# cdcseacave/openMVS

Measured on AMD Instinct MI355X. Metric: Mpix/s depth-map output at 1920x1080 N-view, higher is better.
Workload: dtype f32

## Files before the change

### openmvs_amd/csrc/pm_band.hip

```cpp
#pragma once

#ifndef PM_NDRAW
#define PM_NDRAW 6
#endif
#ifndef PM_BAND_MINWAVES
#define PM_BAND_MINWAVES 3
#endif
#ifndef PM_BAND_MINWAVES_PHOTO
#define PM_BAND_MINWAVES_PHOTO 4
#endif

struct alignas(16) PMPix {
	float nb[2][5];
	float depth, nx, ny, nz, conf;
	float p0, p1, scaleRange, depthRange;
	int st, it, idxScale, flags;
	float hd, hnx, hny, hnz, hp0, hp1;
	int hst, pad0;
	float qX[4][3], qn[4][3];
	float vx, vy, normSq0, sumW;
	double X0x, X0y;
	int x, y;
	float x1[2];
	double hr[3];
	float dr[PM_NDRAW][3];
};
#if defined(__HIP_DEVICE_COMPILE__)
#define PM_LDS __attribute__((address_space(3)))
template <class T> __device__ __forceinline__ PM_LDS T* pm_launder(T* p) { PM_LDS T* q = (PM_LDS T*)p; asm volatile("" : "+v"(q)); return q; }
#else
#define PM_LDS
template <class T> __device__ __forceinline__ T* pm_launder(T* p) { return p; }
#endif
static_assert(sizeof(PMPix) == 368, "sixteen of them, the weights and the views' matrices fit a sixteenth of a CU's LDS (tests/test_kernel_resources.py)");
__device__ __forceinline__ PM_LDS float* pm_pix_sf(PM_LDS PMPix* P) { return P->nb[0]; }
enum { PMF_SMOOTH = 1, PMF_CHANGED = 2, PMF_POK0 = 4, PMF_POK1 = 8 };

template <int G, int VPL, bool GEO, bool BUF, bool TILED>
__device__ __forceinline__ void pm_visit(const PMTask& t, const PMKParams& kp, const PMImgBuf& rs, uint32_t pass, int sgn, float2* s_wg, PMPix* s_pixg, const double* hotBase,
		int g, int v, bool active, int x, int y, int ySafe, size_t idx, const bool* bok, const int* qxs, const int* qys, const size_t* qis, unsigned oldMask,
		float n0D, float n0N0, float n0N1, float n0N2, float n0C, float n1D, float n1N0, float n1N1, float n1N2, float n1C,
		float& rD, float& rN0, float& rN1, float& rN2, float& rC, bool& wr PM_PROF_ARG) {
	constexpr int NBD = PM_SRC_HOT + (GEO ? PM_SRC_GEO : 0);
	constexpr int PPW = 64 / G;
	const int slot = v & 3;
	const pm_gf gDepth = pm_globw(t.depth), gNormal = pm_globw(t.normal), gConf = pm_globw(t.conf);
	const int yTop = ySafe;
	float oDepth = 0.f, oNx = 0.f, oNy = 0.f, oNz = 0.f, oConf = 2.f, prior = 0.f;
	float myD = 0.f, myN0 = 0.f, myN1 = 0.f, myN2 = 1.f;
	unsigned char maskByte = 1;
	if (active && v < 4) {
		if (v == 0) {
			if (t.prior) prior = pm_glob(t.prior)[idx];
			if (t.mask != nullptr) maskByte = t.mask[idx];
			oDepth = gDepth[idx]; oNx = gNormal[idx * 3]; oNy = gNormal[idx * 3 + 1]; oNz = gNormal[idx * 3 + 2]; oConf = gConf[idx];
			myD = bok[0] ? n0D : 0.f; myN0 = n0N0; myN1 = n0N1; myN2 = n0N2;
		}
		else if (v == 1) { myD = bok[1] ? n1D : 0.f; myN0 = n1N0; myN1 = n1N1; myN2 = n1N2; }
		else {
			const size_t qi = slot == 2 ? qis[2] : qis[3];
			const bool old = TILED && ((oldMask >> slot) & 1u);
			const pm_gcf sD = pm_glob(old ? t.depthOld : t.depth), sN = pm_glob(old ? t.normalOld : t.normal);
// ... 103 lines not shown
					else {
						const PmPhilox4 r = pm_philox4x32_10((uint32_t)px, (uint32_t)py, (uint32_t)(PM_STREAM_REFINE * 256) + it, 0u, t.k0, k1);
						e0 = 2.f * pm_u32_to_unit(r.v[0]) - 1.f; e1 = 2.f * pm_u32_to_unit(r.v[1]) - 1.f; e2 = 2.f * pm_u32_to_unit(r.v[2]) - 1.f;
					}
					++it;
					const float ndepth = P->depth + (depthRange * scaleRange) * e0;
					if (!pm_in_range(ndepth, t.dMin, t.dMax)) continue;
					hp0 = p0 + (kp.angle1Range * scaleRange) * e1;
					hp1 = p1 + (kp.angle2Range * scaleRange) * e2;
					pm_dir2normal_vm<PPW>(hp0, hp1, v, hnx, hny, hnz);
					if (hnx * vx + hny * vy + hnz * vz >= 0) continue;
					hd = ndepth;
					need = true; hst = ST_REFINE;
				}
			}
			double hr0 = 0.0, hr1 = 0.0, hr2 = 0.0;
			if (need) pm_homography_plane(P->X0x, P->X0y, hd, hnx, hny, hnz, hr0, hr1, hr2);
			__builtin_amdgcn_wave_barrier();
			if (v == 0) {
				P->hr[0] = hr0; P->hr[1] = hr1; P->hr[2] = hr2;
				P->st = st; P->it = (int)it; P->idxScale = (int)idxScale; P->flags = flags;
				P->scaleRange = scaleRange; P->depthRange = depthRange; P->p0 = p0; P->p1 = p1;
				P->hd = hd; P->hnx = hnx; P->hny = hny; P->hnz = hnz; P->hp0 = hp0; P->hp1 = hp1; P->hst = hst;
			}
		}
		const unsigned long long needBal = __ballot(need);
		if (needBal == 0ull) break;
		PM_TICK(1); PM_COUNT(8, __popcll(needBal)); PM_HIST(__popcll(needBal) / G);
		typename std::conditional<GEO, PMGeoReq, PMNoGeoReq>::type greq[GEO ? VPL : 1];
		if constexpr (GEO) {
			const PM_LDS PMPix* P = pm_launder(s_pixg);
			const double gX0x = P->X0x, gX0y = P->X0y;
#pragma unroll
			for (int u = 0; u < VPL; ++u) {
				const int vw = v + u * G;
				PM_CENSUS_GEO(vw);
				pm_geo_request(need && vw < t.nSrc, hotBase + vw * NBD + PM_SRC_HOT, gX0x, gX0y, hd, greq[u]);
			}
			PM_CENSUS_GEO(-1);
			PM_GEO_HOLD();
		}
		{
			PM_LDS PMPix* P = pm_launder(s_pixg);
			const int flags = P->flags;
			const bool on = need && v < 4 && (flags & PMF_SMOOTH) && ((flags >> (8 + slot)) & 1);
			float myF = 1.f;
// ... 3 lines not shown
				const float planeD = -hd * (hnx * vx + hny * vy + hnz * 1.f);
				const float dist = (hnx * q0 + (hny * q1 + hnz * q2)) + planeD;
				const float r = dist / hd;
				const float factorDepth = pm_expf((r * r) * kp.smoothSigmaDepth);
				const float ca = pm_clampf((hnx * m0 + hny * m1 + hnz * m2) / pm_sqrtf((hnx * hnx + hny * hny + hnz * hnz) * (m0 * m0 + m1 * m1 + m2 * m2)), -1.f, 1.f);
				const float ac = pm_acosf(ca);
				const float factorNormal = pm_expf((ac * ac) * kp.smoothSigmaNormal);
				myF = (1.f - kp.smoothBonusDepth * factorDepth) * (1.f - kp.smoothBonusNormal * factorNormal);
			}
			if (v < 4) pm_pix_sf(P)[slot] = myF;
			__builtin_amdgcn_wave_barrier();
		}
		PM_TICK(2);
		float sc = PM_INF, sc2 = PM_INF;
		{
			const PM_LDS PMPix* P = pm_launder(s_pixg);
#pragma unroll 1
			for (int u = 0; u < VPL; ++u) {
				const int vw = v + u * G;
				if (need && vw < t.nSrc) {
					PM_CENSUS_VIEW(t.w, G, u);
					float s1;
					if constexpr (GEO) s1 = pm_score_view<GEO, BUF ? 2 : 1, true, true>(t.src[vw], t, kp, P->x, P->y, P->X0x, P->X0y, P->normSq0, P->sumW, s_wg, hd, hnx, hny, hnz, 1.f, 1.f, 1.f, 1.f, 0.f,
						hotBase + vw * NBD, hotBase + vw * NBD + PM_SRC_HOT, rs PM_PROF_PASS, (const double*)P->hr, (const float*)pm_pix_sf((PM_LDS PMPix*)P), greq, u, VPL);
					else s1 = pm_score_view<GEO, BUF ? 2 : 1, true, true>(t.src[vw], t, kp, P->x, P->y, P->X0x, P->X0y, P->normSq0, P->sumW, s_wg, hd, hnx, hny, hnz, 1.f, 1.f, 1.f, 1.f, 0.f,
						hotBase + vw * NBD, hotBase + vw * NBD + PM_SRC_HOT, rs PM_PROF_PASS, (const double*)P->hr, (const float*)pm_pix_sf((PM_LDS PMPix*)P));
					PM_CENSUS_VIEW_END();
					if (s1 < sc) { sc2 = sc; sc = s1; } else if (s1 < sc2) sc2 = s1;
				}
			}
		}
		const float nconf = pm_aggregate_vm<G>(sc, t.nSrc, kp.thRobust, sc2);
		{
			PM_LDS PMPix* P = pm_launder(s_pixg);
			if (need && v == 0 && P->conf > nconf) {
				P->conf = nconf; P->depth = P->hd; P->nx = P->hnx; P->ny = P->hny; P->nz = P->hnz;
				int flags = P->flags | PMF_CHANGED;
				P->flags = flags;
				const int hst = P->hst;
				if (hst == ST_RAND) { if (nconf < kp.thConfRand) P->st = ST_DECIDE; }
				else if (hst == ST_REFINE) { P->p0 = P->hp0; P->p1 = P->hp1; const int is = P->idxScale + 1; P->idxScale = is; P->scaleRange = pm_pow2neg((unsigned)is); }
			}
		}
		__builtin_amdgcn_wave_barrier();
		PM_TICK(6);
	}
	{
		const PM_LDS PMPix* P = pm_launder(s_pixg);
		wr = (P->flags & PMF_CHANGED) && valid;
		rD = wr ? P->depth : oDepth; rN0 = wr ? P->nx : oNx; rN1 = wr ? P->ny : oNy; rN2 = wr ? P->nz : oNz; rC = wr ? P->conf : oConf;
	}
}

template <int G, int VPL, bool GEO, bool BUF, bool TILED>
__global__ __launch_bounds__(64, (GEO ? PM_BAND_MINWAVES : PM_BAND_MINWAVES_PHOTO)) void pm_sweep2_kernel(const PMTask* __restrict__ tasks, PMKParams kp, PMStep st, uint32_t pass) {
	constexpr int PPW = 64 / G;
	constexpr int NV = G * VPL;
	constexpr int NBD = PM_SRC_HOT + (GEO ? PM_SRC_GEO : 0);
	static_assert(G >= 4, "a pixel gets at least a quad of lanes");
	PM_PROF_DECL;
	__shared__ float2 s_w[PPW][PM_NT + 1];
	__shared__ double s_src[NV * NBD];
	__shared__ PMPix s_pix[PPW];
	unsigned vbx = blockIdx.x, vby = blockIdx.y;
	{
		const unsigned nbx = gridDim.x, nwg = nbx * gridDim.y, orig = blockIdx.y * nbx + blockIdx.x;
		const unsigned xcd = orig % 8u, q = nwg / 8u, r = nwg % 8u;
		const unsigned wgid = (xcd < r ? xcd * (q + 1u) : r * (q + 1u) + (xcd - r) * q) + orig / 8u;
		vby = wgid / nbx; vbx = wgid - vby * nbx;
	}
	const PMTask& t = tasks[vby];
	const PMImgBuf rs = pm_make_imgbuf(t);
	const int lane = threadIdx.x;
	for (int i = lane; i < NV * NBD; i += 64) {
		double e = ((const double*)&t.src[i / NBD])[i % NBD];
		if constexpr (GEO) if (i % NBD == PM_SRC_HOT + 12) {
			const PMSrcView& sv = t.src[i / NBD];
			const float4* q = sv.depth != nullptr ? pm_task_geoq(t) + sv.dqBase : nullptr;
			e = *(const double*)&q;
		}
		s_src[i] = e;
	}
	const int g = lane % PPW, v = lane / PPW;
	const int w = t.w, h = t.h;
	const PMStepPix sp = pm_step_pixel<TILED>(st, w, h, (int)vbx * PPW + g);
	const bool active = sp.active;
	const int x = sp.x, y = sp.y;
	const size_t idx = (size_t)y * w + x;
	const int sgn = st.dir == 0 ? -1 : 1;
	bool bok[4]; int qxs[4], qys[4]; size_t qis[4];
#pragma unroll
	for (int k = 0; k < 4; ++k) {
		const int ox = (k == 0) ? sgn : (k == 2 ? -sgn : 0), oy = (k == 1) ? sgn : (k == 3 ? -sgn : 0);
		bool ok;
		if (ox == -1) ok = x > PM_HW; else if (ox == 1) ok = x < w - PM_HW; else if (oy == -1) ok = y > PM_HW; else ok = y < h - PM_HW;
		bok[k] = ok && active; qxs[k] = x + ox; qys[k] = y + oy;
		qis[k] = bok[k] ? (size_t)(y + oy) * w + (x + ox) : idx;
	}
	const pm_gf gDepth = pm_globw(t.depth), gNormal = pm_globw(t.normal), gConf = pm_globw(t.conf);
	float n0D = 0.f, n0N0 = 0.f, n0N1 = 0.f, n0N2 = 0.f, n0C = 2.f, n1D = 0.f, n1N0 = 0.f, n1N1 = 0.f, n1N2 = 0.f, n1C = 2.f;
	if (active && v < 2) {
		const size_t q0 = qis[0], q1 = qis[1];
		if (TILED) {
			const pm_gcf nD0 = pm_glob((sp.oldMask & 1u) ? t.depthOld : t.depth), nN0 = pm_glob((sp.oldMask & 1u) ? t.normalOld : t.normal), nC0 = pm_glob((sp.oldMask & 1u) ? t.confOld : t.conf);
			const pm_gcf nD1 = pm_glob((sp.oldMask & 2u) ? t.depthOld : t.depth), nN1 = pm_glob((sp.oldMask & 2u) ? t.normalOld : t.normal), nC1 = pm_glob((sp.oldMask & 2u) ? t.confOld : t.conf);
			if (v == 0) { n0D = nD0[q0]; n0N0 = nN0[q0 * 3]; n0N1 = nN0[q0 * 3 + 1]; n0N2 = nN0[q0 * 3 + 2]; n0C = nC0[q0]; }
			else { n1D = nD1[q1]; n1N0 = nN1[q1 * 3]; n1N1 = nN1[q1 * 3 + 1]; n1N2 = nN1[q1 * 3 + 2]; n1C = nC1[q1]; }
		} else {
			if (v == 0) { n0D = gDepth[q0]; n0N0 = gNormal[q0 * 3]; n0N1 = gNormal[q0 * 3 + 1]; n0N2 = gNormal[q0 * 3 + 2]; n0C = gConf[q0]; }
			else { n1D = gDepth[q1]; n1N0 = gNormal[q1 * 3]; n1N1 = gNormal[q1 * 3 + 1]; n1N2 = gNormal[q1 * 3 + 2]; n1C = gConf[q1]; }
		}
	}
	__syncthreads();
	float rD, rN0, rN1, rN2, rC; bool wr;
	pm_visit<G, VPL, GEO, BUF, TILED>(t, kp, rs, pass, sgn, s_w[g], &s_pix[g], s_src, g, v, active, x, y, active ? y : PM_HW, active ? idx : (size_t)PM_HW * w + PM_HW, bok, qxs, qys, qis, sp.oldMask,
		n0D, n0N0, n0N1, n0N2, n0C, n1D, n1N0, n1N1, n1N2, n1C, rD, rN0, rN1, rN2, rC, wr PM_PROF_PASS);
	if (wr && v == 0) { gDepth[idx] = rD; gNormal[idx * 3] = rN0; gNormal[idx * 3 + 1] = rN1; gNormal[idx * 3 + 2] = rN2; gConf[idx] = rC; }
	PM_PROF_FLUSH();
}
```

### openmvs_amd/csrc/pm_kernels.hip

```cpp
#pragma once
#include <hip/hip_runtime.h>
#include <cstddef>
#include <type_traits>
#include "pm_math.h"

#define PM_MAX_SRC 16
#ifndef PM_BLOCK
#define PM_BLOCK 64
#endif
typedef const float __attribute__((address_space(1)))* pm_gcf;
typedef float __attribute__((address_space(1)))* pm_gf;
#if defined(__HIP_DEVICE_COMPILE__)
typedef float pm_f4v __attribute__((ext_vector_type(4)));
typedef const pm_f4v __attribute__((address_space(1)))* pm_gcf4;
__device__ __forceinline__ pm_gcf4 pm_glob4(const float4* p) { return (pm_gcf4)p; }
__device__ __forceinline__ pm_f4v pm_loadq(pm_gcf4 base, unsigned off) { return base[off]; }
#else
typedef const float4* pm_gcf4;
__device__ __forceinline__ pm_gcf4 pm_glob4(const float4* p) { return p; }
__device__ __forceinline__ float4 pm_loadq(pm_gcf4 base, unsigned off) { return base[off]; }
#endif
__device__ __forceinline__ pm_gcf pm_glob(const float* p) { return (pm_gcf)p; }
__device__ __forceinline__ pm_gf pm_globw(float* p) { return (pm_gf)p; }
#define PM_HW 4
// ... 84 lines not shown
#define PM_COUNT(i, n) do { _pa.a[i] += (unsigned long long)(n); } while (0)
#define PM_HIST(n) do { const int _n = (n); if ((threadIdx.x & 63) == 0) atomicAdd(&pm_hist[_n > 16 ? 16 : _n], 1ull); } while (0)
#define PM_PROF_FLUSH() do { if ((threadIdx.x & 63) == 0) for (int _i = 0; _i < 16; ++_i) atomicAdd(&pm_prof[_i], _pa.a[_i]); } while (0)
#else
#define PM_PROF_ARG
#define PM_PROF_PASS
#define PM_PROF_DECL do {} while (0)
#define PM_TICK(i) do {} while (0)
#define PM_COUNT(i, n) do {} while (0)
#define PM_HIST(n) do {} while (0)
#define PM_PROF_FLUSH() do {} while (0)
#endif
#define PM_FD2R(d) ((d) * (PM_PI_F / 180.f))

#if defined(__HIP_DEVICE_COMPILE__)
__device__ __forceinline__ int pm_mul24(int a, int b) { return __mul24(a, b); }
#else
__device__ __forceinline__ int pm_mul24(int a, int b) { return (int)((unsigned)a * (unsigned)b); }
#endif
__device__ __forceinline__ bool pm_inside1(float px, float py, int w, int h) {
	return px >= 1.f && py >= 1.f && px <= (float)(w - 2) && py <= (float)(h - 2);
}
__device__ __forceinline__ bool pm_in_range(float d, float lo, float hi) { return lo <= d && d < hi; }

__device__ __forceinline__ void pm_dir2normal(float p0, float p1, float& nx, float& ny, float& nz) {
	float sx, cx, sy, cy;
	pm_sincosf(p0, &sx, &cx); pm_sincosf(p1, &sy, &cy);
	nx = cx * sy; ny = sx * sy; nz = cy;
}
__device__ __forceinline__ void pm_random_normal(float u1, float u2, float vx, float vy, float vz, float& nx, float& ny, float& nz) {
	const float a0 = PM_FD2R(0.f), a1 = PM_FD2R(180.f), b0 = PM_FD2R(90.f), b1 = PM_FD2R(180.f);
	const float p0 = a0 + (a1 - a0) * u1;
	const float p1 = b0 + (b1 - b0) * u2;
	pm_dir2normal(p0, p1, nx, ny, nz);
	if (nx * vx + ny * vy + nz * vz > 0) { nx = -nx; ny = -ny; nz = -nz; }
}
__device__ __forceinline__ void pm_correct_normal(float vx, float vy, float vz, float& nx, float& ny, float& nz) {
	const float cosAngLen = nx * vx + ny * vy + nz * vz;
	if (cosAngLen >= 0) {
		const float nv = pm_sqrtf(vx * vx + vy * vy + vz * vz);
		const float phi = pm_minf((pm_acosf(pm_clampf(cosAngLen / nv, -1.f, 1.f)) - PM_FD2R(90.f)) * 1.01f, -0.001f);
		float a0 = ny * vz - nz * vy, a1 = nz * vx - nx * vz, a2 = nx * vy - ny * vx;
		const float an = pm_sqrtf(a0 * a0 + a1 * a1 + a2 * a2);
		const float ia = 1.f / an;
		a0 *= ia; a1 *= ia; a2 *= ia;
		float s, c; pm_sincosf(phi, &s, &c);
// ... 245 lines not shown
	q0 = i0 < r.count ? r.base[i0] : z; q1 = i1 < r.count ? r.base[i1] : z; q2 = i2 < r.count ? r.base[i2] : z; q3 = i3 < r.count ? r.base[i3] : z; q4 = i4 < r.count ? r.base[i4] : z;
}
template <int LEFT> __device__ __forceinline__ void pm_bufwait5(pm_f4v&, pm_f4v&, pm_f4v&, pm_f4v&, pm_f4v&) {}
__device__ __forceinline__ unsigned pm_mad24(int a, int b, unsigned c) { return (unsigned)(((unsigned)a & 0xffffffu) * ((unsigned)b & 0xffffffu)) + c; }
#endif

#ifndef PM_CENSUS_TRIP
#define PM_CENSUS_TRIP()
#define PM_CENSUS_GEO(vw)
#define PM_CENSUS_VIEW(width, G, u)
#define PM_CENSUS_VIEW_AS(width, G, u, lane)
#define PM_CENSUS_VIEW_END()
#endif
#ifdef PM_PROBE_WIDEN_QUAD_BLOCK
struct PMImgBuf { pm_rsrc rs; bool oneBlock = false; };
#else
struct PMImgBuf { pm_rsrc rs; };
#endif
__device__ __forceinline__ PMImgBuf pm_make_imgbuf(const PMTask& t) {
	PMImgBuf b;
	b.rs = pm_make_rsrc(t.qArr, t.qCount);
	return b;
}

template <bool QUAD>
__device__ __forceinline__ void pm_tap_row_global(const pm_gcf img, int sw, int sh, float h0, float h3, float h6, float X0, float X1, float X2,
		const float2* wrow, float& sum, float& sumSq, float& num, bool& oob)
{
	const int lxMax = sw - 2, lyMax = sh - 2;
	float fxs[5], fys[5];
	unsigned offs[5];
#pragma unroll
	for (int j = 0; j < 5; ++j) {
		float ptx, pty;
		pm_div2(X0, X1, X2, &ptx, &pty);
		oob = oob || !pm_inside1(ptx, pty, sw, sh);
		int lx = (int)ptx, ly = (int)pty;
		fxs[j] = ptx - (float)lx; fys[j] = pty - (float)ly;
		lx = min(max(lx, 0), lxMax); ly = min(max(ly, 0), lyMax);
		offs[j] = QUAD ? 4u * ((unsigned)(lx + ly) * (unsigned)sh + (unsigned)ly) : (unsigned)ly * (unsigned)sw + (unsigned)lx;
		X0 += h0; X1 += h3; X2 += h6;
	}
	float v00[5], v01[5], v10[5], v11[5];
#pragma unroll
	for (int j = 0; j < 5; ++j) {
		const pm_gcf p = img + offs[j];
		if (QUAD) { v00[j] = p[0]; v01[j] = p[1]; v10[j] = p[2]; v11[j] = p[3]; }
		else { v00[j] = p[0]; v01[j] = p[1]; v10[j] = p[sw]; v11[j] = p[sw + 1]; }
	}
#pragma unroll
	for (int j = 0; j < 5; ++j) {
		const float fx = fxs[j], fx1 = 1.f - fx, fy = fys[j], fy1 = 1.f - fy;
		const float v = (v00[j] * fx1 + v01[j] * fx) * fy1 + (v10[j] * fx1 + v11[j] * fx) * fy;
		const float2 pw = wrow[j];
		const float vw = v * pw.x;
		sum += vw;
		sumSq += v * vw;
		num += v * pw.y;
	}
}

struct PMRowPos { float ptx[5], pty[5]; };
struct PMRowQ { pm_f4v q0, q1, q2, q3, q4; };
struct PMTapRange { int zlo, zhi, plo, pxhi, pyhi; };
__device__ __forceinline__ void pm_range_corner(PMTapRange& rg, float px, float py, float z) {
	const int ix = pm_f2i(px), iy = pm_f2i(py), iz = pm_f2i(z);
	rg.plo = min(rg.plo, min(ix, iy)); rg.pxhi = max(rg.pxhi, ix); rg.pyhi = max(rg.pyhi, iy);
	rg.zlo = min(rg.zlo, iz); rg.zhi = max(rg.zhi, iz);
}
template <bool BUF, bool CORNERS>
__device__ __forceinline__ void pm_row_issue(const PMImgBuf& rs, unsigned qbase, const pm_gcf4 imgQ, int sw, int sh, float h0, float h3, float h6, float X0, float X1, float X2,
		PMRowPos& p, PMRowQ& q, PMTapRange& rg)
{
	unsigned idx[5];
#pragma unroll
	for (int j = 0; j < 5; ++j) {
		pm_div2_inrange(X0, X1, X2, &p.ptx[j], &p.pty[j]);
		const int lx = (int)p.ptx[j], ly = (int)p.pty[j];
		if (BUF) idx[j] = pm_mad24(lx, sh, pm_mad24(ly, sh + 1, qbase));
		else { const int lxc = min(max(lx, 0), sw - 2), lyc = min(max(ly, 0), sh - 2); idx[j] = (unsigned)(lxc + lyc) * (unsigned)sh + (unsigned)lyc; }
		if (CORNERS && (j == 0 || j == 4)) pm_range_corner(rg, p.ptx[j], p.pty[j], X2);
		X0 += h0; X1 += h3; X2 += h6;
	}
#if defined(PM_PROBE_WIDEN_QUAD_BLOCK) && defined(__HIP_DEVICE_COMPILE__)
	if (BUF && rs.oneBlock) {
#pragma unroll
		for (int j = 0; j < 5; ++j) idx[j] = (idx[j] & 3u) | ((unsigned)__builtin_amdgcn_update_dpp((int)idx[j], (int)idx[j], 0x00, 0xf, 0xf, false) & ~3u);
	}
#endif
	if (BUF) pm_bufload5(q.q0, q.q1, q.q2, q.q3, q.q4, idx[0], idx[1], idx[2], idx[3], idx[4], rs.rs);
	else { q.q0 = pm_loadq(imgQ, idx[0]); q.q1 = pm_loadq(imgQ, idx[1]); q.q2 = pm_loadq(imgQ, idx[2]); q.q3 = pm_loadq(imgQ, idx[3]); q.q4 = pm_loadq(imgQ, idx[4]); }
}
template <bool BUF, int LEFT>
__device__ __forceinline__ void pm_row_consume(const PMRowPos& p, PMRowQ& q, const float2* wrow, float& sum, float& sumSq, float& num)
{
	float t00[5], t01[5], t10[5], t11[5];
	if (BUF) pm_bufwait5<LEFT>(q.q0, q.q1, q.q2, q.q3, q.q4);
	const pm_f4v qq[5] = {q.q0, q.q1, q.q2, q.q3, q.q4};
#pragma unroll
	for (int j = 0; j < 5; ++j) { t00[j] = qq[j].x; t01[j] = qq[j].y; t10[j] = qq[j].z; t11[j] = qq[j].w; }
#pragma unroll
	for (int j = 0; j < 5; ++j) {
		const float fx = pm_fract_pos(p.ptx[j]), fx1 = 1.f - fx, fy = pm_fract_pos(p.pty[j]), fy1 = 1.f - fy;
		const float v = (t00[j] * fx1 + t01[j] * fx) * fy1 + (t10[j] * fx1 + t11[j] * fx) * fy;
		const float2 pw = wrow[j];
		const float vw = v * pw.x;
		sum += vw;
		sumSq += v * vw;
		num += v * pw.y;
	}
}
template <bool BUF>
__device__ __forceinline__ void pm_taps_fast(const PMImgBuf& rs, unsigned qbase, const pm_gcf4 imgQ, int sw, int sh, const float* H, float bX0, float bX1, float bX2,
		const float2* wts, float& sum, float& sumSq, float& num, PMTapRange& rg)
{
	PMRowPos pa, pb; PMRowQ qa, qb;
	pm_row_issue<BUF, true>(rs, qbase, imgQ, sw, sh, H[0], H[3], H[6], bX0, bX1, bX2, pa, qa, rg);
#pragma unroll 1
	for (int i = 0; i < 4; i += 2) {
		bX0 += H[1]; bX1 += H[4]; bX2 += H[7];
		pm_row_issue<BUF, false>(rs, qbase, imgQ, sw, sh, H[0], H[3], H[6], bX0, bX1, bX2, pb, qb, rg);
		PM_SCHED_BARRIER();
		pm_row_consume<BUF, 5>(pa, qa, wts + i * 5, sum, sumSq, num);
		PM_SCHED_BARRIER();
		bX0 += H[1]; bX1 += H[4]; bX2 += H[7];
		pm_row_issue<BUF, false>(rs, qbase, imgQ, sw, sh, H[0], H[3], H[6], bX0, bX1, bX2, pa, qa, rg);
		PM_SCHED_BARRIER();
		pm_row_consume<BUF, 5>(pb, qb, wts + (i + 1) * 5, sum, sumSq, num);
		PM_SCHED_BARRIER();
	}
	pm_range_corner(rg, pa.ptx[0], pa.pty[0], bX2);
	pm_range_corner(rg, pa.ptx[4], pa.pty[4], (((bX2 + H[6]) + H[6]) + H[6]) + H[6]);
	pm_row_consume<BUF, 0>(pa, qa, wts + 20, sum, sumSq, num);
}

#if !defined(__HIP_DEVICE_COMPILE__) && defined(PM_DEBUG_REDO)
inline unsigned long long pm_tap_census[2][4];
extern "C" __attribute__((visibility("default"))) void pm_debug_tap_census(unsigned long long out[8], int reset) {
	for (int i = 0; i < 8; ++i) { if (out) out[i] = pm_tap_census[i / 4][i % 4]; if (reset) pm_tap_census[i / 4][i % 4] = 0; }
}
#endif
__device__ __forceinline__ unsigned pm_dq_index(int lx, int ly, int dw, int dh) {
	int d = lx + ly;
	if (d >= dw) { d -= dw; if (d >= dw) d %= dw; }
	return (unsigned)d * (unsigned)dh + (unsigned)ly;
}
struct PMGeoReq {
	pm_f4v q;
	float x1x, x1y, Y2;
	bool has, ok;
};
struct PMNoGeoReq {};
#if defined(__HIP_DEVICE_COMPILE__)
#define PM_GEO_HOLD() asm volatile("" ::: "memory")
#else
#define PM_GEO_HOLD() do {} while (0)
#endif
__device__ __forceinline__ void pm_geo_request(bool on, const double* geoTab, double X0x, double X0y, float depth, PMGeoReq& r) {
	r.has = false; r.ok = false; r.x1x = 0.f; r.x1y = 0.f; r.Y2 = 0.f;
	r.q.x = 0.f; r.q.y = 0.f; r.q.z = 0.f; r.q.w = 0.f;
	if (!on) return;
	const float* gt = (const float*)geoTab;
// ... 32 lines not shown
__device__ __forceinline__ float pm_geo_consistency(float x1x, float x1y, float Y2, float x0y0, float x1y0, float x0y1, float x1y1, const float* Tr, const float* Tn, int x, int y) {
	float consistency = 4.f;
	const int lx = (int)x1x, ly = (int)x1y;
	const float fx = x1x - (float)lx, fx1 = 1.f - fx;
	const float fy = x1y - (float)ly, fy1 = 1.f - fy;
	const bool b00 = pm_fabsf(Y2 - x0y0) / Y2 < 0.03f, b10 = pm_fabsf(Y2 - x1y0) / Y2 < 0.03f;
	const bool b01 = pm_fabsf(Y2 - x0y1) / Y2 < 0.03f, b11 = pm_fabsf(Y2 - x1y1) / Y2 < 0.03f;
	if (b00 || b10 || b01 || b11) {
		const float depth1 =
			fy1 * (fx1 * (b00 ? x0y0 : (b10 ? x1y0 : (b01 ? x0y1 : x1y1))) + fx * (b10 ? x1y0 : (b00 ? x0y0 : (b11 ? x1y1 : x0y1)))) +
			fy  * (fx1 * (b01 ? x0y1 : (b11 ? x1y1 : (b00 ? x0y0 : x1y0))) + fx * (b11 ? x1y1 : (b01 ? x0y1 : (b10 ? x1y0 : x0y0))));
		const float Xd0 = x1x * depth1, Xd1 = x1y * depth1, Xd2 = depth1;
		const float B0 = (Tr[0] * Xd0 + Tr[1] * Xd1 + Tr[2] * Xd2) + Tn[0];
		const float B1 = (Tr[3] * Xd0 + Tr[4] * Xd1 + Tr[5] * Xd2) + Tn[1];
		const float B2 = (Tr[6] * Xd0 + Tr[7] * Xd1 + Tr[8] * Xd2) + Tn[2];
		const float xbx = B0 / B2, xby = B1 / B2;
		const float dx = (float)x - xbx, dy = (float)y - xby;
		const float dist = pm_sqrtf(dx * dx + dy * dy);
		consistency = pm_minf(pm_sqrtf(dist * (dist + 2.f)), consistency);
	}
	return consistency;
}

template <bool GEO, int MODE, bool PF = false, bool EARLY = false>
__device__ __forceinline__ float pm_score_view(const PMSrcView& s, const PMTask& t, const PMKParams& kp,
		int x, int y, double X0x, double X0y, float normSq0, float sumW, const float2* wts,
		float depth, float nx, float ny, float nz,
		float sf0, float sf1, float sf2, float sf3, float prior,
		const double* hot, const double* geoTab, const PMImgBuf& rs PM_PROF_ARG, const double* rpre = nullptr, const float* sfp = nullptr,
		const PMGeoReq* greq = nullptr, int gsel = 0, int gn = 1)
{
	const int sw = ((const int*)(hot + 12))[0], sh = ((const int*)(hot + 12))[1];
	float H[9];
	pm_homography(hot, t, X0x, X0y, depth, nx, ny, nz, H, rpre);
	PM_TICK(3);
	const float px = (float)(x - PM_HW), py = (float)(y - PM_HW);
	const float X0 = H[0] * px + H[1] * py + H[2];
	const float X1 = H[3] * px + H[4] * py + H[5];
	const float X2 = H[6] * px + H[7] * py + H[8];
	float bX0 = X0, bX1 = X1, bX2 = X2;
#pragma unroll
	for (int i = 0; i < 9; ++i) H[i] *= 2.f;
	float sum = 0.f, sumSq = 0.f, num = 0.f;
	bool oob = false;
	if (MODE == 0) {
#pragma unroll 1
		for (int i = 0; i < 5; ++i) {
			pm_tap_row_global<false>(pm_glob(s.img), sw, sh, H[0], H[3], H[6], bX0, bX1, bX2, wts + i * 5, sum, sumSq, num, oob);
			bX0 += H[1]; bX1 += H[4]; bX2 += H[7];
		}
	} else {
		const bool sane = pm_fabsf(X0) + 8.f * (pm_fabsf(H[0]) + pm_fabsf(H[1])) < 5e17f && pm_fabsf(X1) + 8.f * (pm_fabsf(H[3]) + pm_fabsf(H[4])) < 5e17f
			&& pm_fabsf(X2) + 8.f * (pm_fabsf(H[6]) + pm_fabsf(H[7])) < 5e11f;
		if (EARLY && sane) {
			bool outside = false;
			float cx, cy;
			if (bX2 >= 9.094947e-13f && bX2 <= 1.0995116e12f) { pm_div2_inrange(bX0, bX1, bX2, &cx, &cy); outside = !pm_inside1(cx, cy, sw, sh); }
			float c0 = bX0, c1 = bX1, c2 = bX2;
#pragma unroll
			for (int i = 0; i < 4; ++i) { c0 += H[1]; c1 += H[4]; c2 += H[7]; }
#pragma unroll
			for (int j = 0; j < 4; ++j) { c0 += H[0]; c1 += H[3]; c2 += H[6]; }
			if (c2 >= 9.094947e-13f && c2 <= 1.0995116e12f) { pm_div2_inrange(c0, c1, c2, &cx, &cy); outside = outside || !pm_inside1(cx, cy, sw, sh); }
#if !defined(__HIP_DEVICE_COMPILE__) && defined(PM_DEBUG_REDO)
			if (outside) pm_tap_census[PF][3]++;
#endif
			if (outside) return kp.thRobust;
		}
		const unsigned qbase = ((const unsigned*)(hot + 13))[0];
		const pm_gcf4 imgQ = pm_glob4(s.imgQ);
		const float rX0 = bX0, rX1 = bX1, rX2 = bX2;
		PMTapRange rg = {0x7fffffff, (int)0x80000000, 0x7fffffff, (int)0x80000000, (int)0x80000000};
		pm_taps_fast<MODE == 2>(rs, qbase, imgQ, sw, sh, H, bX0, bX1, bX2, wts, sum, sumSq, num, rg);
		const bool exact = sane && rg.zlo >= pm_f2i(9.094947e-13f) && rg.zhi <= pm_f2i(1.0995116e12f);
		const bool cornersIn = rg.plo >= pm_f2i(1.f) && rg.pxhi <= pm_f2i((float)(sw - 2)) && rg.pyhi <= pm_f2i((float)(sh - 2));
		const float delta = (float)max(sw, sh) * 7.62939453125e-06f;
		const bool allIn = rg.plo >= pm_f2i(1.f + delta) && rg.pxhi <= pm_f2i((float)(sw - 2) - delta) && rg.pyhi <= pm_f2i((float)(sh - 2) - delta)
			&& (unsigned)rg.zhi - (unsigned)rg.zlo <= 0x00800000u;
#if !defined(__HIP_DEVICE_COMPILE__) && defined(PM_DEBUG_REDO)
		pm_tap_census[PF][0]++; if (exact && cornersIn && !allIn) pm_tap_census[PF][1]++; if (!exact) pm_tap_census[PF][2]++;
#endif
		if (exact) {
			oob = !cornersIn;
			if (cornersIn && !allIn) {
				float cX0 = rX0, cX1 = rX1, cX2 = rX2;
#pragma unroll 1
				for (int i = 0; i < 5; ++i) {
					float X0t = cX0, X1t = cX1, X2t = cX2;
#pragma unroll 1
					for (int j = 0; j < 5; ++j) {
						float ptx, pty;
						pm_div2_inrange(X0t, X1t, X2t, &ptx, &pty);
						oob = oob || !pm_inside1(ptx, pty, sw, sh);
						X0t += H[0]; X1t += H[3]; X2t += H[6];
					}
					cX0 += H[1]; cX1 += H[4]; cX2 += H[7];
				}
			}
		} else {
			sum = 0.f; sumSq = 0.f; num = 0.f;
			bX0 = rX0; bX1 = rX1; bX2 = rX2;
#pragma unroll 1
			for (int i = 0; i < 5; ++i) {
				pm_tap_row_global<true>(pm_glob((const float*)s.imgQ), sw, sh, H[0], H[3], H[6], bX0, bX1, bX2, wts + i * 5, sum, sumSq, num, oob);
				bX0 += H[1]; bX1 += H[4]; bX2 += H[7];
			}
		}
	}
	PM_TICK(4);
	if (oob) return kp.thRobust;
	const float normSq1 = sumSq - (sum * sum) / sumW;
	const float nrmSq = normSq0 * normSq1;
	if (nrmSq <= 1e-16f) return kp.thRobust;
	const float ncc = pm_clampf(num / pm_sqrtf(nrmSq), -1.f, 1.f);
	float score = 1.f - ncc;
	if (sfp) { sf0 = sfp[0]; sf1 = sfp[1]; sf2 = sfp[2]; sf3 = sfp[3]; }
	score *= sf0; score *= sf1; score *= sf2; score *= sf3;
	if (GEO) {
		if (!greq) {
			const float* gt = (const float*)geoTab;
			const float* sdepth = *(const float* const*)(geoTab + 12);
			const int dw = ((const int*)(geoTab + 13))[0], dh = ((const int*)(geoTab + 13))[1];
			float Tl[9], Tm[3], Tr[9], Tn[3];
#pragma unroll
			for (int i = 0; i < 9; ++i) { Tl[i] = gt[i]; Tr[i] = gt[12 + i]; }
#pragma unroll
			for (int i = 0; i < 3; ++i) { Tm[i] = gt[9 + i]; Tn[i] = gt[21 + i]; }
#pragma unroll
			for (int i = 0; i < 9; ++i) PM_OPAQUE(Tr[i]);
#pragma unroll
			for (int i = 0; i < 3; ++i) PM_OPAQUE(Tn[i]);
			if (sdepth != nullptr) {
// ... 23 lines not shown
#pragma unroll
		for (int i = 0; i < 3; ++i) Tn[i] = gt[21 + i];
#pragma unroll
		for (int i = 0; i < 9; ++i) PM_OPAQUE(Tr[i]);
#pragma unroll
		for (int i = 0; i < 3; ++i) PM_OPAQUE(Tn[i]);
		if (rq.has) {
			float consistency = 4.f;
			const float Y2 = rq.Y2;
			{
				const float x1x = rq.x1x, x1y = rq.x1y;
				if (rq.ok) {
					consistency = pm_geo_consistency(x1x, x1y, Y2, rq.q.x, rq.q.y, rq.q.z, rq.q.w, Tr, Tn, x, y);
				}
			}
			score += kp.geoWeight * consistency;
		}
		}
	}
	if (PF) {
		const float2 pf = wts[PM_NT];
		float pfy = pf.y;
		PM_OPAQUE(pfy);
		if (pf.x > 0) {
			const float deltaDepth = pm_minf(pm_fabsf(pf.x - depth) / pf.x, 0.5f);
			score = (1.f - pfy) * score + pfy * deltaDepth;
		}
	} else if (prior > 0) {
		const float deltaDepth = pm_minf(pm_fabsf(prior - depth) / prior, 0.5f);
		const float sigma = -1.f / (1.f * 0.02f);
		const float f = pm_expf(normSq0 * sigma);
		score = (1.f - f) * score + f * deltaDepth;
	}
	PM_TICK(5);
	return pm_minf(2.f, score);
}

template <int G>
__device__ __forceinline__ float pm_aggregate(float viewScore, int nSrc, float thRobust, float viewScore2 = PM_INF) {
	float m1, m2;
	pm_group_min2<G>(viewScore, viewScore2, m1, m2);
	if (nSrc <= 1) return m1;
	if (m2 >= thRobust) return m1;
	return (m1 + m2) / 2.f;
}

__device__ __forceinline__ int pm_fold(int d, int w) { if (d >= w) { d -= w; if (d >= w) d %= w; } return d; }
template <int G, bool SKEW>
__device__ __forceinline__ void pm_fill_patch(const PMTask& t, bool inb, int x, int y, int v, float2* wts, float& normSq0, float& sumW) {
	const float sigmaColor = -1.f / (2.f * (0.1f * 0.1f));
	const float sigmaSpatial = -1.f / (2.f * 9.f);
	if (inb) {
// ... 58 lines not shown
	const pm_gf gDepth = pm_globw(t.depth), gNormal = pm_globw(t.normal), gConf = pm_globw(t.conf);
	const float prior = t.prior ? pm_glob(t.prior)[idx] : 0.f;
	const bool masked = t.mask != nullptr && t.mask[idx] == 0;
	const bool valid = inb && !masked && !(normSq0 < kp.thMagnitudeSq && !(prior > 0));
	if (!valid) {
		if (v == 0) { gDepth[idx] = 0.f; gNormal[idx * 3] = 0.f; gNormal[idx * 3 + 1] = 0.f; gNormal[idx * 3 + 2] = 0.f; gConf[idx] = 2.f; }
		return;
	}
	const double X0x = ((double)x - t.cx) / t.fx, X0y = ((double)y - t.cy) / t.fy;
	const float vx = (float)X0x, vy = (float)X0y, vz = 1.f;
	float depth = gDepth[idx];
	float nx = gNormal[idx * 3], ny = gNormal[idx * 3 + 1], nz = gNormal[idx * 3 + 2];
	const PmPhilox4 r = pm_philox4x32_10((uint32_t)x, (uint32_t)y, (uint32_t)(PM_STREAM_INIT * 256), 0u, t.k0, t.k1base + pass);
	if (!pm_in_range(depth, t.dMin, t.dMax)) {
		const float rr = t.dMinSqr + (t.dMaxSqr - t.dMinSqr) * pm_u32_to_unit(r.v[0]);
		depth = rr * rr;
		pm_random_normal(pm_u32_to_unit(r.v[1]), pm_u32_to_unit(r.v[2]), vx, vy, vz, nx, ny, nz);
	} else if (nx * vx + ny * vy + nz * vz >= 0) {
		pm_random_normal(pm_u32_to_unit(r.v[1]), pm_u32_to_unit(r.v[2]), vx, vy, vz, nx, ny, nz);
	}
	float sc = PM_INF, sc2 = PM_INF;
	PM_PROF_DECL;
	const PMImgBuf rs = MODE == 2 ? pm_make_imgbuf(t) : PMImgBuf();
#pragma unroll 1
	for (int u = 0; u < VPL; ++u) {
		const int vw = v + u * G;
		if (vw < t.nSrc) {
			const float s1 = pm_score_view<GEO, MODE>(t.src[vw], t, kp, x, y, X0x, X0y, normSq0, sumW, s_w[g], depth, nx, ny, nz, 1.f, 1.f, 1.f, 1.f, prior, t.src[vw].Hl, (const double*)t.src[vw].Tl,
				rs PM_PROF_PASS);
			if (s1 < sc) { sc2 = sc; sc = s1; } else if (s1 < sc2) sc2 = s1;
		}
	}
	const float conf = pm_aggregate<G>(sc, t.nSrc, kp.thRobust, sc2);
	if (v == 0) { gDepth[idx] = depth; gNormal[idx * 3] = nx; gNormal[idx * 3 + 1] = ny; gNormal[idx * 3 + 2] = nz; gConf[idx] = conf; }
}

template <bool GEO, bool BUF>
__global__ __launch_bounds__(64, PM_WIDE_MINWAVES) void pm_sweep_wide_kernel(const PMTask* __restrict__ tasks, PMKParams kp, int dir, int d, int xlo, int count, uint32_t pass) {
	constexpr int G = 8;
	constexpr int NBD = PM_SRC_HOT + (GEO ? PM_SRC_GEO : 0);
	PM_PROF_DECL;
	__shared__ float2 s_w[PM_NT + 1];
	__shared__ double s_src[G * NBD];
	const PMTask& t = tasks[blockIdx.y];
	const PMImgBuf rs = pm_make_imgbuf(t);
	const int lane = threadIdx.x, c = lane >> 3, v = lane & 7;
	for (int i = lane; i < G * NBD; i += 64) s_src[i] = ((const double*)&t.src[i / NBD])[i % NBD];
	const double* hot = s_src + v * NBD;
	const int w = t.w, h = t.h;
	const int x = xlo + (int)blockIdx.x, y = d - x;
	const size_t idx = (size_t)y * w + x;
	const pm_gf gDepth = pm_globw(t.depth), gNormal = pm_globw(t.normal), gConf = pm_globw(t.conf);
// ... 349 lines not shown
```

Baseline: 60.76.

## Fuse early out-of-bounds test into first tap row and hoist level bounds

Moves the early out-of-image rejection from a separate corner projection into the first row issue of the tap loop, so the corner positions already computed there are reused and the gathers are skipped when a corner falls outside. Hoists the source-level bounds (width, height, margins) into a wave-uniform struct built once per kernel via readfirstlane instead of recomputing them per view. Precomputes the prior depth delta once per pixel in LDS so each view's scoring reads it instead of recomputing a divide. It also changes the output write index to read pixel coordinates from LDS and adds several probe macros and debug counters.

New measurement: 61.96 (median of 6 runs). +2.0%, better.

```diff
diff --git a/openmvs_amd/csrc/pm_band.hip b/openmvs_amd/csrc/pm_band.hip
--- a/openmvs_amd/csrc/pm_band.hip
+++ b/openmvs_amd/csrc/pm_band.hip
@@ -16,7 +16,8 @@
 	float p0, p1, scaleRange, depthRange;
 	int st, it, idxScale, flags;
 	float hd, hnx, hny, hnz, hp0, hp1;
-	int hst, pad0;
+	int hst;
+	float hdd;
 	float qX[4][3], qn[4][3];
 	float vx, vy, normSq0, sumW;
 	double X0x, X0y;
@@ -37,7 +38,7 @@
 enum { PMF_SMOOTH = 1, PMF_CHANGED = 2, PMF_POK0 = 4, PMF_POK1 = 8 };
 
 template <int G, int VPL, bool GEO, bool BUF, bool TILED>
-__device__ __forceinline__ void pm_visit(const PMTask& t, const PMKParams& kp, const PMImgBuf& rs, uint32_t pass, int sgn, float2* s_wg, PMPix* s_pixg, const double* hotBase,
+__device__ __forceinline__ void pm_visit(const PMTask& t, const PMKParams& kp, const PMImgBuf& rs, const PMLvl& lv, uint32_t pass, int sgn, float2* s_wg, PMPix* s_pixg, const double* hotBase,
 		int g, int v, bool active, int x, int y, int ySafe, size_t idx, const bool* bok, const int* qxs, const int* qys, const size_t* qis, unsigned oldMask,
 		float n0D, float n0N0, float n0N1, float n0N2, float n0C, float n1D, float n1N0, float n1N1, float n1N2, float n1C,
 		float& rD, float& rN0, float& rN1, float& rN2, float& rC, bool& wr PM_PROF_ARG) {
@@ -187,6 +188,10 @@
 				P->st = st; P->it = (int)it; P->idxScale = (int)idxScale; P->flags = flags;
 				P->scaleRange = scaleRange; P->depthRange = depthRange; P->p0 = p0; P->p1 = p1;
 				P->hd = hd; P->hnx = hnx; P->hny = hny; P->hnz = hnz; P->hp0 = hp0; P->hp1 = hp1; P->hst = hst;
+				if (t.prior) {
+					const float pr = s_wg[PM_NT].x;
+					P->hdd = (need && pr > 0) ? pm_prior_delta(pr, hd) : 0.f;
+				}
 			}
 		}
 		const unsigned long long needBal = __ballot(need);
@@ -236,9 +241,9 @@
 					PM_CENSUS_VIEW(t.w, G, u);
 					float s1;
 					if constexpr (GEO) s1 = pm_score_view<GEO, BUF ? 2 : 1, true, true>(t.src[vw], t, kp, P->x, P->y, P->X0x, P->X0y, P->normSq0, P->sumW, s_wg, hd, hnx, hny, hnz, 1.f, 1.f, 1.f, 1.f, 0.f,
-						hotBase + vw * NBD, hotBase + vw * NBD + PM_SRC_HOT, rs PM_PROF_PASS, (const double*)P->hr, (const float*)pm_pix_sf((PM_LDS PMPix*)P), greq, u, VPL);
+						hotBase + vw * NBD, hotBase + vw * NBD + PM_SRC_HOT, rs PM_PROF_PASS, (const double*)P->hr, (const float*)pm_pix_sf((PM_LDS PMPix*)P), greq, u, VPL, BUF ? &lv : nullptr, (const float*)&P->hdd);
 					else s1 = pm_score_view<GEO, BUF ? 2 : 1, true, true>(t.src[vw], t, kp, P->x, P->y, P->X0x, P->X0y, P->normSq0, P->sumW, s_wg, hd, hnx, hny, hnz, 1.f, 1.f, 1.f, 1.f, 0.f,
-						hotBase + vw * NBD, hotBase + vw * NBD + PM_SRC_HOT, rs PM_PROF_PASS, (const double*)P->hr, (const float*)pm_pix_sf((PM_LDS PMPix*)P));
+						hotBase + vw * NBD, hotBase + vw * NBD + PM_SRC_HOT, rs PM_PROF_PASS, (const double*)P->hr, (const float*)pm_pix_sf((PM_LDS PMPix*)P), nullptr, 0, 1, BUF ? &lv : nullptr, (const float*)&P->hdd);
 					PM_CENSUS_VIEW_END();
 					if (s1 < sc) { sc2 = sc; sc = s1; } else if (s1 < sc2) sc2 = s1;
 				}
@@ -285,6 +290,7 @@
 	}
 	const PMTask& t = tasks[vby];
 	const PMImgBuf rs = pm_make_imgbuf(t);
+	const PMLvl lv = BUF ? pm_make_lvl(t) : PMLvl();
 	const int lane = threadIdx.x;
 	for (int i = lane; i < NV * NBD; i += 64) {
 		double e = ((const double*)&t.src[i / NBD])[i % NBD];
@@ -327,8 +333,12 @@
 	}
 	__syncthreads();
 	float rD, rN0, rN1, rN2, rC; bool wr;
-	pm_visit<G, VPL, GEO, BUF, TILED>(t, kp, rs, pass, sgn, s_w[g], &s_pix[g], s_src, g, v, active, x, y, active ? y : PM_HW, active ? idx : (size_t)PM_HW * w + PM_HW, bok, qxs, qys, qis, sp.oldMask,
+	pm_visit<G, VPL, GEO, BUF, TILED>(t, kp, rs, lv, pass, sgn, s_w[g], &s_pix[g], s_src, g, v, active, x, y, active ? y : PM_HW, active ? idx : (size_t)PM_HW * w + PM_HW, bok, qxs, qys, qis, sp.oldMask,
 		n0D, n0N0, n0N1, n0N2, n0C, n1D, n1N0, n1N1, n1N2, n1C, rD, rN0, rN1, rN2, rC, wr PM_PROF_PASS);
-	if (wr && v == 0) { gDepth[idx] = rD; gNormal[idx * 3] = rN0; gNormal[idx * 3 + 1] = rN1; gNormal[idx * 3 + 2] = rN2; gConf[idx] = rC; }
+	if (wr && v == 0) {
+		const PM_LDS PMPix* P = pm_launder(&s_pix[g]);
+		const size_t io = (size_t)P->y * w + P->x;
+		gDepth[io] = rD; gNormal[io * 3] = rN0; gNormal[io * 3 + 1] = rN1; gNormal[io * 3 + 2] = rN2; gConf[io] = rC;
+	}
 	PM_PROF_FLUSH();
 }
diff --git a/openmvs_amd/csrc/pm_kernels.hip b/openmvs_amd/csrc/pm_kernels.hip
--- a/openmvs_amd/csrc/pm_kernels.hip
+++ b/openmvs_amd/csrc/pm_kernels.hip
@@ -130,6 +130,20 @@
 	return px >= 1.f && py >= 1.f && px <= (float)(w - 2) && py <= (float)(h - 2);
 }
 __device__ __forceinline__ bool pm_in_range(float d, float lo, float hi) { return lo <= d && d < hi; }
+struct PMLvl {
+	int sw, sh;
+	float xm, ym;
+	float oneD;
+	float xmD, ymD;
+};
+__device__ __forceinline__ PMLvl pm_lvl_of(int sw, int sh) {
+	PMLvl l;
+	l.sw = sw; l.sh = sh; l.xm = (float)(sw - 2); l.ym = (float)(sh - 2);
+	const float delta = (float)max(sw, sh) * 7.62939453125e-06f;
+	l.oneD = 1.f + delta; l.xmD = l.xm - delta; l.ymD = l.ym - delta;
+	return l;
+}
+__device__ __forceinline__ bool pm_inside1(float px, float py, const PMLvl& l) { return px >= 1.f && py >= 1.f && px <= l.xm && py <= l.ym; }
 
 __device__ __forceinline__ void pm_dir2normal(float p0, float p1, float& nx, float& ny, float& nz) {
 	float sx, cx, sy, cy;
@@ -421,6 +435,19 @@
 	b.rs = pm_make_rsrc(t.qArr, t.qCount);
 	return b;
 }
+#if defined(__HIP_DEVICE_COMPILE__)
+__device__ __forceinline__ int pm_uniform(int v) { return __builtin_amdgcn_readfirstlane(v); }
+#else
+__device__ __forceinline__ int pm_uniform(int v) { return v; }
+#endif
+__device__ __forceinline__ float pm_uniform(float v) { return pm_u2f((uint32_t)pm_uniform(pm_f2i(v))); }
+__device__ __forceinline__ PMLvl pm_make_lvl(const PMTask& t) {
+	const PMLvl l = pm_lvl_of(t.src[0].w, t.src[0].h);
+	PMLvl u;
+	u.sw = pm_uniform(l.sw); u.sh = pm_uniform(l.sh); u.xm = pm_uniform(l.xm); u.ym = pm_uniform(l.ym);
+	u.oneD = pm_uniform(l.oneD); u.xmD = pm_uniform(l.xmD); u.ymD = pm_uniform(l.ymD);
+	return u;
+}
 
 template <bool QUAD>
 __device__ __forceinline__ void pm_tap_row_global(const pm_gcf img, int sw, int sh, float h0, float h3, float h6, float X0, float X1, float X2,
@@ -467,11 +494,13 @@
 	rg.plo = min(rg.plo, min(ix, iy)); rg.pxhi = max(rg.pxhi, ix); rg.pyhi = max(rg.pyhi, iy);
 	rg.zlo = min(rg.zlo, iz); rg.zhi = max(rg.zhi, iz);
 }
-template <bool BUF, bool CORNERS>
-__device__ __forceinline__ void pm_row_issue(const PMImgBuf& rs, unsigned qbase, const pm_gcf4 imgQ, int sw, int sh, float h0, float h3, float h6, float X0, float X1, float X2,
-		PMRowPos& p, PMRowQ& q, PMTapRange& rg)
+template <bool BUF, bool CORNERS, bool EARLY = false>
+__device__ __forceinline__ bool pm_row_issue(const PMImgBuf& rs, unsigned qbase, const pm_gcf4 imgQ, const PMLvl& lv, float h0, float h3, float h6, float X0, float X1, float X2,
+		PMRowPos& p, PMRowQ& q, PMTapRange& rg, bool early = false)
 {
+	const int sw = lv.sw, sh = lv.sh;
 	unsigned idx[5];
+	bool outside = false;
 #pragma unroll
 	for (int j = 0; j < 5; ++j) {
 		pm_div2_inrange(X0, X1, X2, &p.ptx[j], &p.pty[j]);
@@ -479,8 +508,15 @@
 		if (BUF) idx[j] = pm_mad24(lx, sh, pm_mad24(ly, sh + 1, qbase));
 		else { const int lxc = min(max(lx, 0), sw - 2), lyc = min(max(ly, 0), sh - 2); idx[j] = (unsigned)(lxc + lyc) * (unsigned)sh + (unsigned)lyc; }
 		if (CORNERS && (j == 0 || j == 4)) pm_range_corner(rg, p.ptx[j], p.pty[j], X2);
+#ifdef PM_PROBE_EVAL_TRIM
+		if (CORNERS && EARLY && j == 0)
+#else
+		if (CORNERS && EARLY && (j == 0 || j == 4))
+#endif
+			outside = outside || (X2 >= 9.094947e-13f && X2 <= 1.0995116e12f && !pm_inside1(p.ptx[j], p.pty[j], lv));
 		X0 += h0; X1 += h3; X2 += h6;
 	}
+	if (CORNERS && EARLY && early && outside) return true;
 #if defined(PM_PROBE_WIDEN_QUAD_BLOCK) && defined(__HIP_DEVICE_COMPILE__)
 	if (BUF && rs.oneBlock) {
 #pragma unroll
@@ -489,6 +525,7 @@
 #endif
 	if (BUF) pm_bufload5(q.q0, q.q1, q.q2, q.q3, q.q4, idx[0], idx[1], idx[2], idx[3], idx[4], rs.rs);
 	else { q.q0 = pm_loadq(imgQ, idx[0]); q.q1 = pm_loadq(imgQ, idx[1]); q.q2 = pm_loadq(imgQ, idx[2]); q.q3 = pm_loadq(imgQ, idx[3]); q.q4 = pm_loadq(imgQ, idx[4]); }
+	return false;
 }
 template <bool BUF, int LEFT>
 __device__ __forceinline__ void pm_row_consume(const PMRowPos& p, PMRowQ& q, const float2* wrow, float& sum, float& sumSq, float& num)
@@ -509,21 +546,21 @@
 		num += v * pw.y;
 	}
 }
-template <bool BUF>
-__device__ __forceinline__ void pm_taps_fast(const PMImgBuf& rs, unsigned qbase, const pm_gcf4 imgQ, int sw, int sh, const float* H, float bX0, float bX1, float bX2,
-		const float2* wts, float& sum, float& sumSq, float& num, PMTapRange& rg)
+template <bool BUF, bool EARLY>
+__device__ __forceinline__ bool pm_taps_fast(const PMImgBuf& rs, unsigned qbase, const pm_gcf4 imgQ, const PMLvl& lv, const float* H, float bX0, float bX1, float bX2,
+		const float2* wts, float& sum, float& sumSq, float& num, PMTapRange& rg, bool early)
 {
 	PMRowPos pa, pb; PMRowQ qa, qb;
-	pm_row_issue<BUF, true>(rs, qbase, imgQ, sw, sh, H[0], H[3], H[6], bX0, bX1, bX2, pa, qa, rg);
+	if (pm_row_issue<BUF, true, EARLY>(rs, qbase, imgQ, lv, H[0], H[3], H[6], bX0, bX1, bX2, pa, qa, rg, early)) return true;
 #pragma unroll 1
 	for (int i = 0; i < 4; i += 2) {
 		bX0 += H[1]; bX1 += H[4]; bX2 += H[7];
-		pm_row_issue<BUF, false>(rs, qbase, imgQ, sw, sh, H[0], H[3], H[6], bX0, bX1, bX2, pb, qb, rg);
+		pm_row_issue<BUF, false>(rs, qbase, imgQ, lv, H[0], H[3], H[6], bX0, bX1, bX2, pb, qb, rg);
 		PM_SCHED_BARRIER();
 		pm_row_consume<BUF, 5>(pa, qa, wts + i * 5, sum, sumSq, num);
 		PM_SCHED_BARRIER();
 		bX0 += H[1]; bX1 += H[4]; bX2 += H[7];
-		pm_row_issue<BUF, false>(rs, qbase, imgQ, sw, sh, H[0], H[3], H[6], bX0, bX1, bX2, pa, qa, rg);
+		pm_row_issue<BUF, false>(rs, qbase, imgQ, lv, H[0], H[3], H[6], bX0, bX1, bX2, pa, qa, rg);
 		PM_SCHED_BARRIER();
 		pm_row_consume<BUF, 5>(pb, qb, wts + (i + 1) * 5, sum, sumSq, num);
 		PM_SCHED_BARRIER();
@@ -531,12 +568,17 @@
 	pm_range_corner(rg, pa.ptx[0], pa.pty[0], bX2);
 	pm_range_corner(rg, pa.ptx[4], pa.pty[4], (((bX2 + H[6]) + H[6]) + H[6]) + H[6]);
 	pm_row_consume<BUF, 0>(pa, qa, wts + 20, sum, sumSq, num);
+	return false;
 }
 
 #if !defined(__HIP_DEVICE_COMPILE__) && defined(PM_DEBUG_REDO)
 inline unsigned long long pm_tap_census[2][4];
 extern "C" __attribute__((visibility("default"))) void pm_debug_tap_census(unsigned long long out[8], int reset) {
 	for (int i = 0; i < 8; ++i) { if (out) out[i] = pm_tap_census[i / 4][i % 4]; if (reset) pm_tap_census[i / 4][i % 4] = 0; }
+}
+inline unsigned long long pm_tap_census_outside[2];
+extern "C" __attribute__((visibility("default"))) void pm_debug_tap_census_outside(unsigned long long out[2], int reset) {
+	for (int i = 0; i < 2; ++i) { if (out) out[i] = pm_tap_census_outside[i]; if (reset) pm_tap_census_outside[i] = 0; }
 }
 #endif
 __device__ __forceinline__ unsigned pm_dq_index(int lx, int ly, int dw, int dh) {
@@ -615,15 +657,18 @@
 	return consistency;
 }
 
+__device__ __forceinline__ float pm_prior_delta(float prior, float depth) { return pm_minf(pm_fabsf(prior - depth) / prior, 0.5f); }
+
 template <bool GEO, int MODE, bool PF = false, bool EARLY = false>
 __device__ __forceinline__ float pm_score_view(const PMSrcView& s, const PMTask& t, const PMKParams& kp,
 		int x, int y, double X0x, double X0y, float normSq0, float sumW, const float2* wts,
 		float depth, float nx, float ny, float nz,
 		float sf0, float sf1, float sf2, float sf3, float prior,
 		const double* hot, const double* geoTab, const PMImgBuf& rs PM_PROF_ARG, const double* rpre = nullptr, const float* sfp = nullptr,
-		const PMGeoReq* greq = nullptr, int gsel = 0, int gn = 1)
+		const PMGeoReq* greq = nullptr, int gsel = 0, int gn = 1, const PMLvl* lvu = nullptr, const float* ddp = nullptr)
 {
-	const int sw = ((const int*)(hot + 12))[0], sh = ((const int*)(hot + 12))[1];
+	const PMLvl lv = lvu ? *lvu : pm_lvl_of(((const int*)(hot + 12))[0], ((const int*)(hot + 12))[1]);
+	const int sw = lv.sw, sh = lv.sh;
 	float H[9];
 	pm_homography(hot, t, X0x, X0y, depth, nx, ny, nz, H, rpre);
 	PM_TICK(3);
@@ -645,30 +690,43 @@
 	} else {
 		const bool sane = pm_fabsf(X0) + 8.f * (pm_fabsf(H[0]) + pm_fabsf(H[1])) < 5e17f && pm_fabsf(X1) + 8.f * (pm_fabsf(H[3]) + pm_fabsf(H[4])) < 5e17f
 			&& pm_fabsf(X2) + 8.f * (pm_fabsf(H[6]) + pm_fabsf(H[7])) < 5e11f;
-		if (EARLY && sane) {
-			bool outside = false;
-			float cx, cy;
-			if (bX2 >= 9.094947e-13f && bX2 <= 1.0995116e12f) { pm_div2_inrange(bX0, bX1, bX2, &cx, &cy); outside = !pm_inside1(cx, cy, sw, sh); }
-			float c0 = bX0, c1 = bX1, c2 = bX2;
-#pragma unroll
-			for (int i = 0; i < 4; ++i) { c0 += H[1]; c1 += H[4]; c2 += H[7]; }
-#pragma unroll
-			for (int j = 0; j < 4; ++j) { c0 += H[0]; c1 += H[3]; c2 += H[6]; }
-			if (c2 >= 9.094947e-13f && c2 <= 1.0995116e12f) { pm_div2_inrange(c0, c1, c2, &cx, &cy); outside = outside || !pm_inside1(cx, cy, sw, sh); }
-#if !defined(__HIP_DEVICE_COMPILE__) && defined(PM_DEBUG_REDO)
-			if (outside) pm_tap_census[PF][3]++;
-#endif
-			if (outside) return kp.thRobust;
-		}
 		const unsigned qbase = ((const unsigned*)(hot + 13))[0];
 		const pm_gcf4 imgQ = pm_glob4(s.imgQ);
 		const float rX0 = bX0, rX1 = bX1, rX2 = bX2;
 		PMTapRange rg = {0x7fffffff, (int)0x80000000, 0x7fffffff, (int)0x80000000, (int)0x80000000};
-		pm_taps_fast<MODE == 2>(rs, qbase, imgQ, sw, sh, H, bX0, bX1, bX2, wts, sum, sumSq, num, rg);
+#ifdef PM_PROBE_EARLY_OPPOSITE
+		if (EARLY && sane) {
+			bool outside = false;
+			float cx, cy;
+			if (bX2 >= 9.094947e-13f && bX2 <= 1.0995116e12f) { pm_div2_inrange(bX0, bX1, bX2, &cx, &cy); outside = !pm_inside1(cx, cy, lv); }
+			float c0 = bX0, c1 = bX1, c2 = bX2;
+#pragma unroll
+			for (int i = 0; i < 4; ++i) { c0 += H[1]; c1 += H[4]; c2 += H[7]; }
+#pragma unroll
+			for (int j = 0; j < 4; ++j) { c0 += H[0]; c1 += H[3]; c2 += H[6]; }
+			if (c2 >= 9.094947e-13f && c2 <= 1.0995116e12f) { pm_div2_inrange(c0, c1, c2, &cx, &cy); outside = outside || !pm_inside1(cx, cy, lv); }
+#if !defined(__HIP_DEVICE_COMPILE__) && defined(PM_DEBUG_REDO)
+			if (outside) pm_tap_census[PF][3]++;
+#endif
+			if (outside) return kp.thRobust;
+		}
+		constexpr bool EARLY_ = false;
+#elif defined(PM_PROBE_NO_EARLY)
+		constexpr bool EARLY_ = false;
+#else
+		constexpr bool EARLY_ = EARLY;
+#endif
+		const bool outsideEarly = pm_taps_fast<MODE == 2, EARLY_>(rs, qbase, imgQ, lv, H, bX0, bX1, bX2, wts, sum, sumSq, num, rg, sane);
+#if !defined(__HIP_DEVICE_COMPILE__) && defined(PM_DEBUG_REDO)
+		if (outsideEarly) pm_tap_census[PF][3]++;
+#endif
+		if (outsideEarly) return kp.thRobust;
 		const bool exact = sane && rg.zlo >= pm_f2i(9.094947e-13f) && rg.zhi <= pm_f2i(1.0995116e12f);
-		const bool cornersIn = rg.plo >= pm_f2i(1.f) && rg.pxhi <= pm_f2i((float)(sw - 2)) && rg.pyhi <= pm_f2i((float)(sh - 2));
-		const float delta = (float)max(sw, sh) * 7.62939453125e-06f;
-		const bool allIn = rg.plo >= pm_f2i(1.f + delta) && rg.pxhi <= pm_f2i((float)(sw - 2) - delta) && rg.pyhi <= pm_f2i((float)(sh - 2) - delta)
+		int swp = sw, shp = sh;
+		if (!lvu && EARLY) { PM_OPAQUE(swp); PM_OPAQUE(shp); }
+		const PMLvl lp = lvu ? lv : pm_lvl_of(swp, shp);
+		const bool cornersIn = rg.plo >= pm_f2i(1.f) && rg.pxhi <= pm_f2i(lp.xm) && rg.pyhi <= pm_f2i(lp.ym);
+		const bool allIn = rg.plo >= pm_f2i(lp.oneD) && rg.pxhi <= pm_f2i(lp.xmD) && rg.pyhi <= pm_f2i(lp.ymD)
 			&& (unsigned)rg.zhi - (unsigned)rg.zlo <= 0x00800000u;
 #if !defined(__HIP_DEVICE_COMPILE__) && defined(PM_DEBUG_REDO)
 		pm_tap_census[PF][0]++; if (exact && cornersIn && !allIn) pm_tap_census[PF][1]++; if (!exact) pm_tap_census[PF][2]++;
@@ -684,7 +742,7 @@
 					for (int j = 0; j < 5; ++j) {
 						float ptx, pty;
 						pm_div2_inrange(X0t, X1t, X2t, &ptx, &pty);
-						oob = oob || !pm_inside1(ptx, pty, sw, sh);
+						oob = oob || !pm_inside1(ptx, pty, lp);
 						X0t += H[0]; X1t += H[3]; X2t += H[6];
 					}
 					cX0 += H[1]; cX1 += H[4]; cX2 += H[7];
@@ -701,6 +759,9 @@
 		}
 	}
 	PM_TICK(4);
+#if !defined(__HIP_DEVICE_COMPILE__) && defined(PM_DEBUG_REDO)
+	if (MODE != 0 && oob) pm_tap_census_outside[PF]++;
+#endif
 	if (oob) return kp.thRobust;
 	const float normSq1 = sumSq - (sum * sum) / sumW;
 	const float nrmSq = normSq0 * normSq1;
@@ -770,12 +831,14 @@
 		const float2 pf = wts[PM_NT];
 		float pfy = pf.y;
 		PM_OPAQUE(pfy);
+#ifndef PM_PROBE_EVAL_TRIM
 		if (pf.x > 0) {
-			const float deltaDepth = pm_minf(pm_fabsf(pf.x - depth) / pf.x, 0.5f);
+			const float deltaDepth = ddp ? *ddp : pm_prior_delta(pf.x, depth);
 			score = (1.f - pfy) * score + pfy * deltaDepth;
 		}
+#endif
 	} else if (prior > 0) {
-		const float deltaDepth = pm_minf(pm_fabsf(prior - depth) / prior, 0.5f);
+		const float deltaDepth = pm_prior_delta(prior, depth);
 		const float sigma = -1.f / (1.f * 0.02f);
 		const float f = pm_expf(normSq0 * sigma);
 		score = (1.f - f) * score + f * deltaDepth;
@@ -880,12 +943,13 @@
 	float sc = PM_INF, sc2 = PM_INF;
 	PM_PROF_DECL;
 	const PMImgBuf rs = MODE == 2 ? pm_make_imgbuf(t) : PMImgBuf();
+	const PMLvl lv = MODE == 2 ? pm_make_lvl(t) : PMLvl();
 #pragma unroll 1
 	for (int u = 0; u < VPL; ++u) {
 		const int vw = v + u * G;
 		if (vw < t.nSrc) {
 			const float s1 = pm_score_view<GEO, MODE>(t.src[vw], t, kp, x, y, X0x, X0y, normSq0, sumW, s_w[g], depth, nx, ny, nz, 1.f, 1.f, 1.f, 1.f, prior, t.src[vw].Hl, (const double*)t.src[vw].Tl,
-				rs PM_PROF_PASS);
+				rs PM_PROF_PASS, nullptr, nullptr, nullptr, 0, 1, MODE == 2 ? &lv : nullptr);
 			if (s1 < sc) { sc2 = sc; sc = s1; } else if (s1 < sc2) sc2 = s1;
 		}
 	}
```
